# Andurdur/Chroma-Subsampling-Image-Compressor

Hardware: NVIDIA B200
Metric: input megapixels/s (higher is better)
Workload: dtype u8

## Files before the change

chroma-subsampling-image-compressor_b200/csrc/csic_flex_kernel.cu:

```cuda
#include <cuda_runtime.h>

#include <cstdint>
#include <type_traits>

#include "csic_internal.h"
#include "csic_device_math.cuh"
#include "csic_tma.cuh"

namespace csic {

namespace {

constexpr uint32_t kCtaWideSpan = 2048u;
constexpr uint32_t kDirectRowBytes = 257u;

__device__ __forceinline__ void sts64(uint32_t a, uint32_t x, uint32_t y) {
  asm volatile("st.shared.v2.u32 [%0], {%1, %2};" ::"r"(a), "r"(x), "r"(y) : "memory");
}
__device__ __forceinline__ void sts128(uint32_t a, uint32_t x, uint32_t y, uint32_t z, uint32_t w) {
  asm volatile("st.shared.v4.u32 [%0], {%1, %2, %3, %4};" ::"r"(a), "r"(x), "r"(y), "r"(z), "r"(w) : "memory");
}
__device__ __forceinline__ uint32_t ldg8_now(const uint8_t* p) {
  uint32_t v;
  asm volatile("ld.global.nc.u8 %0, [%1];" : "=r"(v) : "l"(p));
  return v;
}

__device__ __forceinline__ bool pow2_divides(uint32_t n, uint32_t m) {
  return n != 0u && (n & (n - 1u)) == 0u && (m & (m - 1u)) == 0u && n <= m;
}

template <typename F>
__device__ __forceinline__ void for_each_span(uint32_t n, uint32_t len, uint32_t NC, F&& fn) {
  const uint32_t tid = threadIdx.x, NW = NC >> 5;
  if ((len >= kCtaWideSpan || n == 1) && pow2_divides(n, NW)) {
    const uint32_t sh = 31u - __clz(NW) - (31u - __clz(n));
    const uint32_t parts = 1u << sh, j = (tid >> 5) >> sh, part = (tid >> 5) & (parts - 1u);
    fn(j, part * 32u + (tid & 31u), parts * 32u);
  } else if (len >= kCtaWideSpan || n == 1) {
    for (uint32_t j = 0; j < n; ++j) fn(j, tid, NC);
  } else {
    for (uint32_t j = tid >> 5; j < n; j += NW) fn(j, tid & 31u, 32u);
  }
}

__device__ __forceinline__ uint32_t lds_px(uint32_t a) {
  const uint32_t b = a & ~3u;
  return __funnelshift_r(lds32(b), lds32(b + 4), (a & 3u) * 8u);
}

template <uint32_t PXB>
__device__ __forceinline__ void load_granule_any(uint32_t a, uint32_t pxb, uint32_t (&p)[4]) {
  const uint32_t b = a & ~3u, sh = (a & 3u) * 8u;
  if (PXB == 3u) {
    const uint32_t w0 = lds32(b), w1 = lds32(b + 4), w2 = lds32(b + 8), w3 = lds32(b + 12);
    const uint32_t v0 = __funnelshift_r(w0, w1, sh), v1 = __funnelshift_r(w1, w2, sh), v2 = __funnelshift_r(w2, w3, sh);
    p[0] = v0;
    p[1] = __funnelshift_r(v0, v1, 24);
    p[2] = __funnelshift_r(v1, v2, 16);
    p[3] = v2 >> 8;
  } else if (PXB == 6u) {
    const uint32_t w0 = lds32(b), w1 = lds32(b + 4), w2 = lds32(b + 8), w3 = lds32(b + 12), w4 = lds32(b + 16), w5 = lds32(b + 20);
    p[0] = __funnelshift_r(w0, w1, sh);
    p[1] = __funnelshift_r(__funnelshift_r(w1, w2, sh), __funnelshift_r(w2, w3, sh), 16);
    p[2] = __funnelshift_r(w3, w4, sh);
    p[3] = __funnelshift_r(__funnelshift_r(w4, w5, sh), w5 >> sh, 16);
  } else {
#pragma unroll
    for (int j = 0; j < 4; ++j) p[j] = __funnelshift_r(lds32(b + j * pxb), lds32(b + j * pxb + 4), sh);
  }
}

template <int FMT> struct FlexFmt {
  static constexpr uint32_t kUnit = (FMT == KF_YCC888 || FMT == KF_RGB888) ? 12u : (FMT == KF_SLOT32 ? 16u : (FMT == KF_SLOT16 ? 8u : 4u));
};

struct FlexDesc {
  uint32_t k, ro0, nrows, col0;
  uint32_t npx, a0, gpr, last_px;
  uint32_t obase_lo, obase_hi, st_mul, st_add;
  uint32_t mode, sh, magic, n_gran;
  uint32_t row_out, out_one, ncols, direct;
};
static_assert(sizeof(FlexDesc) == kFlexDescBytes, "kFlexDescBytes out of sync");

}

template <int FMT, bool TRUNC, uint32_t HFE, uint32_t PXB, bool DIRECT>
__device__ __forceinline__ void flex_consume(const KPlan& P, uint8_t* smem, const Ring& ring) {
  constexpr uint32_t kUnit = FlexFmt<FMT>::kUnit;
  const uint32_t tid = threadIdx.x, NC = blockDim.x - 32u, NW = NC >> 5;
  const uint32_t sbase = smem_u32(smem), out_s = sbase + P.out_buf_off, held_base = sbase + P.meta_off;
  const uint32_t desc0 = sbase + P.bar_off + kRingBarBytes * ring.S;
  const uint32_t in_stage = P.stage_stride * (uint32_t)P.tile_rows + 32u;
  const uint32_t ipb = (uint32_t)P.in_px_bytes, pxb = (uint32_t)P.f * ipb;
  const uint32_t nsplit = (uint32_t)P.nsplit;
  const bool vhold = P.vf == 2;
  const uint32_t my = P.qmask & 0xFFu, mcb = (P.qmask >> 8) & 0xFFu, mcr = (P.qmask >> 16) & 0xFFu;
  const uint32_t qm0 = my | (mcb << 8) | (mcr << 16) | (my << 24);
  const uint32_t qm1 = mcb | (mcr << 8) | (my << 16) | (mcb << 24);
  const uint32_t qm2 = mcr | (my << 8) | (mcb << 16) | (mcr << 24);
  const int shy = 8 + P.sy, shb = 8 + P.scb, shr = 8 + P.scr, ly = P.cb_bits + P.cr_bits, lb = P.cr_bits;
  const bool q8 = FMT == KF_SLOT32 && P.sy == 0 && P.scb == 0 && P.scr == 0;
  const uint32_t vs_sh = P.planar_vs == 2 ? 1u : 0u, hs_sh = P.planar_hs == 4 ? 2u : (P.planar_hs == 2 ? 1u : 0u);
  const uint32_t rs_mul = P.in_dense ? P.in_row_bytes : P.stage_stride;
  const uint32_t rs_add = P.in_dense ? 0u : (((uint32_t)P.row_step * P.in_row_bytes) & 15u);

  Ring::Pos pos;
  for (uint32_t it = 0; it < ring.n_my; ++it, pos.next(ring.S)) {
    const uint32_t s = pos.s;
    ring.wait_full(pos);
    const uint32_t da = desc0 + s * kFlexDescBytes;
    const uint4 d0 = lds128(da), d1 = lds128(da + 16u), d2 = lds128(da + 32u), d3 = lds128(da + 48u);
    const uint4 d4 = lds128(da + 64u);
    const uint32_t Dk = d0.x, Dro0 = d0.y, Dnrows = d0.z, Dcol0 = d0.w, Dnpx = d1.x, Da0 = d1.y;
    constexpr bool direct = DIRECT;
    consumer_barrier(NC);

    const uint32_t in_s = sbase + s * in_stage, held_s = held_base + s * (uint32_t)kFlexMaxRows * 4u;
    const uint32_t gpr = d1.z, last_px = d1.w;
    uint8_t* obase = reinterpret_cast<uint8_t*>((uint64_t)d2.x | ((uint64_t)d2.y << 32));
    const uint32_t oa0 = d2.x, st_mul = d2.z, st_add = d2.w;
    uint8_t* fout = P.out + (uint64_t)Dk * P.out_frame_bytes;
    const uint32_t c_first = (Dro0 + (1u << vs_sh) - 1u) >> vs_sh;
    const uint32_t c_last1 = ((Dro0 + Dnrows - 1u) >> vs_sh) + 1u;
    const uint32_t nrc = (FMT == KF_PLANAR && c_last1 > c_first) ? c_last1 - c_first : 0u;
    const uint32_t ccols = (Dnpx + (1u << hs_sh) - 1u) >> hs_sh;
    const uint32_t cb_s = out_s + Dnrows * st_mul + 16u, cr_s = cb_s + nrc * ccols;

    auto granule = [&](uint32_t row, uint32_t g, uint32_t rs, uint32_t so_row, uint32_t hv) {
      const uint32_t c = g * 4u;
      uint32_t p[4], dy[4], xb[4], xr[4];
      if (c + 3u <= last_px) {
        load_granule_any<PXB>(rs + c * pxb, pxb, p);
      } else {
#pragma unroll
        for (int j = 0; j < 4; ++j) p[j] = lds_px(rs + min(c + j, last_px) * pxb);
      }
#pragma unroll
      for (int j = 0; j < 4; ++j) dy[j] = fwd_y16(p[j], P.coef_y);
      const uint32_t so = so_row + g * kUnit;
      uint8_t* gp = obase + (uint64_t)row * P.out_row_bytes + g * kUnit;
      const uint32_t gbytes = min(kUnit, d4.x - g * kUnit);
      if (FMT == KF_RGB888) {
        const uint32_t my8 = my << 8, mcb8 = mcb << 8, mcr8 = mcr << 8;
        auto emit = [&](const InvChroma& t0, const InvChroma& t1, const InvChroma& t2, const InvChroma& t3) {
          uint32_t w0, w1, w2;
        inv_granule(dy, my8, t0, t1, t2, t3, w0, w1, w2);
          if (direct) { const uint32_t ww[3] = {w0, w1, w2}; direct_store(gp, ww, gbytes); }
          else { sts32(so, w0); sts32(so + 4, w1); sts32(so + 8, w2); }
        };
        if (hv) {
          const InvChroma t = inv_chroma_terms(fwd_nc16<TRUNC>(hv & 0x00FFFFFFu, P.coef_ncb), fwd_nc16<TRUNC>(hv & 0x00FFFFFFu, P.coef_ncr), mcb8, mcr8);
          emit(t, t, t, t);
        } else {
          InvChroma t[4];
#pragma unroll
          for (int j = 0; j < 4; j += (int)HFE) t[j] = inv_chroma_terms(fwd_nc16<TRUNC>(p[j], P.coef_ncb), fwd_nc16<TRUNC>(p[j], P.coef_ncr), mcb8, mcr8);
          emit(t[0], t[1 - 1 % HFE], t[2 - 2 % HFE], t[3 - 3 % HFE]);
        }
        return;
      }
      if (hv) {
        const uint32_t hb = fwd_nc16<TRUNC>(hv & 0x00FFFFFFu, P.coef_ncb), hr = fwd_nc16<TRUNC>(hv & 0x00FFFFFFu, P.coef_ncr);
#pragma unroll
        for (int j = 0; j < 4; ++j) { xb[j] = hb; xr[j] = hr; }
      } else {
        xb[0] = fwd_nc16<TRUNC>(p[0], P.coef_ncb); xr[0] = fwd_nc16<TRUNC>(p[0], P.coef_ncr);
        if (HFE == 1) { xb[1] = fwd_nc16<TRUNC>(p[1], P.coef_ncb); xr[1] = fwd_nc16<TRUNC>(p[1], P.coef_ncr); }
        else { xb[1] = xb[0]; xr[1] = xr[0]; }
        if (HFE <= 2) { xb[2] = fwd_nc16<TRUNC>(p[2], P.coef_ncb); xr[2] = fwd_nc16<TRUNC>(p[2], P.coef_ncr); }
        else { xb[2] = xb[0]; xr[2] = xr[0]; }
        if (HFE == 1) { xb[3] = fwd_nc16<TRUNC>(p[3], P.coef_ncb); xr[3] = fwd_nc16<TRUNC>(p[3], P.coef_ncr); }
        else { xb[3] = xb[2]; xr[3] = xr[2]; }
      }
      if (FMT == KF_YCC888) {
        uint32_t t, u, ww[3];
        t = __byte_perm(dy[0], xb[0], 0x0051); u = __byte_perm(xr[0], dy[1], 0x0051);
        ww[0] = (__byte_perm(t, u, 0x5410) ^ 0x00FFFF00u) & qm0;
        t = __byte_perm(xb[1], xr[1], 0x0051); u = __byte_perm(dy[2], xb[2], 0x0051);
        ww[1] = (__byte_perm(t, u, 0x5410) ^ 0xFF00FFFFu) & qm1;
        t = __byte_perm(xr[2], dy[3], 0x0051); u = __byte_perm(xb[3], xr[3], 0x0051);
        ww[2] = (__byte_perm(t, u, 0x5410) ^ 0xFFFF00FFu) & qm2;
        if (direct) direct_store(gp, ww, gbytes);
        else { sts32(so, ww[0]); sts32(so + 4, ww[1]); sts32(so + 8, ww[2]); }
      } else if (FMT == KF_PLANAR) {
        const uint32_t my4 = my * 0x01010101u;
        sts32(so, __byte_perm(__byte_perm(dy[0], dy[1], 0x0051), __byte_perm(dy[2], dy[3], 0x0051), 0x5410) & my4);
        if (!hv) {
          const uint32_t crow = (((Dro0 + row) >> vs_sh) - c_first) * ccols + (c >> hs_sh);
          if (HFE == 1) {
#pragma unroll
            for (int j = 0; j < 4; ++j)
              if (c + j <= last_px) { sts8(cb_s + crow + j, (~(xb[j] >> 8)) & mcb); sts8(cr_s + crow + j, (~(xr[j] >> 8)) & mcr); }
          } else if (HFE == 2) {
            sts8(cb_s + crow, (~(xb[0] >> 8)) & mcb); sts8(cr_s + crow, (~(xr[0] >> 8)) & mcr);
            if (c + 2 <= last_px) { sts8(cb_s + crow + 1, (~(xb[2] >> 8)) & mcb); sts8(cr_s + crow + 1, (~(xr[2] >> 8)) & mcr); }
          } else {
            sts8(cb_s + crow, (~(xb[0] >> 8)) & mcb); sts8(cr_s + crow, (~(xr[0] >> 8)) & mcr);
          }
        }
      } else {
        uint32_t v[4];
        if (q8) {
#pragma unroll
          for (int j = 0; j < 4; ++j)
            v[j] = __byte_perm(__byte_perm(xr[j], xb[j], 0x0051), dy[j], 0x7510) ^ 0x0000FFFFu;
        } else {
#pragma unroll
          for (int j = 0; j < 4; ++j)
            v[j] = ((dy[j] >> shy) << ly) | (((xb[j] ^ 0xFFFFu) >> shb) << lb) | ((xr[j] ^ 0xFFFFu) >> shr);
        }
        if (c + 3u > last_px) {
#pragma unroll
          for (int j = 0; j < 4; ++j) if (c + j > last_px) v[j] = 0u;
        }
        if (direct) {
          if (FMT == KF_SLOT32) direct_store(gp, v, gbytes);
          else if (FMT == KF_SLOT16) { const uint32_t ww[2] = {v[0] | (v[1] << 16), v[2] | (v[3] << 16)}; direct_store(gp, ww, gbytes); }
          else { const uint32_t ww[1] = {v[0] | (v[1] << 8) | (v[2] << 16) | (v[3] << 24)}; direct_store(gp, ww, gbytes); }
        } else if (FMT == KF_SLOT32) {
          if ((so & 15u) == 0) sts128(so, v[0], v[1], v[2], v[3]);
          else if ((so & 7u) == 0) { sts64(so, v[0], v[1]); sts64(so + 8, v[2], v[3]); }
          else { sts32(so, v[0]); sts32(so + 4, v[1]); sts32(so + 8, v[2]); sts32(so + 12, v[3]); }
        } else if (FMT == KF_SLOT16) {
          if ((so & 7u) == 0) sts64(so, v[0] | (v[1] << 16), v[2] | (v[3] << 16));
          else { sts32(so, v[0] | (v[1] << 16)); sts32(so + 4, v[2] | (v[3] << 16)); }
        } else {
          sts32(so, v[0] | (v[1] << 8) | (v[2] << 16) | (v[3] << 24));
        }
      }
    };
    auto row_in = [&](uint32_t row) { return in_s + row * rs_mul + ((Da0 + row * rs_add) & 15u); };
    auto row_st = [&](uint32_t row) { return out_s + row * st_mul + ((oa0 + row * st_add) & 12u); };
    if (d3.x == 0u) {
      const uint32_t parts = 1u << d3.y, row = (tid >> 5) >> d3.y, part = (tid >> 5) & (parts - 1u);
      if (row < Dnrows) {
        const uint32_t rs = row_in(row), so_row = row_st(row), hv = vhold ? lds32(held_s + row * 4u) : 0u;
        for (uint32_t g = part * 32u + (tid & 31u); g < gpr; g += parts * 32u) granule(row, g, rs, so_row, hv);
      }
    } else if (d3.x == 1u) {
      for (uint32_t row = 0; row < Dnrows; ++row) {
        const uint32_t rs = row_in(row), so_row = row_st(row), hv = vhold ? lds32(held_s + row * 4u) : 0u;
        for (uint32_t g = tid; g < gpr; g += NC) granule(row, g, rs, so_row, hv);
      }
    } else if (d3.x == 2u) {
      for (uint32_t row = tid >> 5; row < Dnrows; row += NW) {
        const uint32_t rs = row_in(row), so_row = row_st(row), hv = vhold ? lds32(held_s + row * 4u) : 0u;
        for (uint32_t g = tid & 31u; g < gpr; g += 32u) granule(row, g, rs, so_row, hv);
      }
    } else {
      for (uint32_t q = tid; q < d3.w; q += NC) {
        const uint32_t row = gpr > 1u ? __umulhi(q, d3.z) : q, g = q - row * gpr;
        granule(row, g, row_in(row), row_st(row), vhold ? lds32(held_s + row * 4u) : 0u);
      }
    }
    consumer_barrier(NC);
    if (tid == 0) mbar_arrive(ring.empty(s));

    if (direct) {
    } else if (d4.y) {
      span_store(obase, out_s + (oa0 & 12u), Dnrows * d4.x, tid, NC);
    } else {
      for_each_span(Dnrows, d4.x, NC, [&](uint32_t j, uint32_t t, uint32_t n) {
        span_store(obase + (uint64_t)j * P.out_row_bytes, out_s + j * st_mul + ((oa0 + j * st_add) & 12u), d4.x, t, n);
      });
    }
    if (FMT == KF_PLANAR && nrc) {
      const uint64_t coff = (uint64_t)c_first * (uint32_t)P.planar_cw + (Dcol0 >> hs_sh);
      uint8_t* cb_g = fout + P.planar_cb_off + coff;
      uint8_t* cr_g = fout + P.planar_cr_off + coff;
      if (nsplit == 1) {
        span_store(cb_g, cb_s, nrc * ccols, tid, NC);
        span_store(cr_g, cr_s, nrc * ccols, tid, NC);
      } else {
        for_each_span(nrc, ccols, NC, [&](uint32_t j, uint32_t t, uint32_t n) {
          span_store(cb_g + (uint64_t)j * (uint32_t)P.planar_cw, cb_s + j * ccols, ccols, t, n);
          span_store(cr_g + (uint64_t)j * (uint32_t)P.planar_cw, cr_s + j * ccols, ccols, t, n);
        });
      }
    }
  }
}

template <int FMT, bool TRUNC>
__global__ void __launch_bounds__(kFlexMaxThreads, 4) csic_flex_kernel(const __grid_constant__ KPlan P) {
  extern __shared__ __align__(128) uint8_t smem[];
  constexpr uint32_t kUnit = FlexFmt<FMT>::kUnit, kOpx = kUnit / 4u;
  const uint32_t tid = threadIdx.x, NT = blockDim.x;
  const uint32_t sbase = smem_u32(smem), held_base = sbase + P.meta_off;
  const uint32_t in_stage = P.stage_stride * (uint32_t)P.tile_rows + 32u;
  const uint32_t ipb = (uint32_t)P.in_px_bytes, f = (uint32_t)P.f, pxb = f * ipb;
  const uint32_t nsplit = (uint32_t)P.nsplit;
  const uint32_t hfe = (uint32_t)P.hfe;
  const bool vhold = P.vf == 2;
  const uint64_t rstep = (uint64_t)(uint32_t)P.row_step * P.in_row_bytes;
  const Ring ring(sbase + P.bar_off, (uint32_t)P.stages, P.n_tiles);
  if (ring.n_my == 0) return;
  const uint32_t rs_mul = P.in_dense ? P.in_row_bytes : P.stage_stride;
  const uint32_t NC = NT - 32u;
  ring.init(1);

  if (tid >= NC) {
    const uint32_t lane = tid - NC;
    const uint64_t pol = policy_evict_first();
    const uint32_t t2 = blockIdx.x / nsplit, g2 = gridDim.x / nsplit;
    uint32_t pseg = blockIdx.x - t2 * nsplit, pk = t2 / P.tiles_per_band, ptb = t2 - pk * P.tiles_per_band;
    const uint32_t dseg = gridDim.x - g2 * nsplit, dk = g2 / P.tiles_per_band, dtb = g2 - dk * P.tiles_per_band;
    const uintptr_t lim_lo = reinterpret_cast<uintptr_t>(P.in) + (uint64_t)((uint32_t)P.row0 * (uint32_t)P.row_step) * P.in_row_bytes;
    const uintptr_t lim_hi = reinterpret_cast<uintptr_t>(P.in) + (uint64_t)(P.n_frames - 1u) * P.in_frame_bytes +
                             (uint64_t)((uint32_t)(P.row0 + P.band_rows - 1) * (uint32_t)P.row_step) * P.in_row_bytes +
                             ((uint32_t)P.Wo - 1u) * pxb + ipb;
    Ring::Pos pos;
    for (uint32_t j = 0; j < ring.n_my; ++j, pos.next(ring.S)) {
      const uint32_t s = pos.s, bar = ring.full(s), in_s = sbase + s * in_stage;
      ring.wait_empty(pos, j);
      FlexDesc* d = reinterpret_cast<FlexDesc*>(smem + P.bar_off + kRingBarBytes * ring.S) + s;
      const uint32_t ro0 = (uint32_t)P.row0 + ptb * (uint32_t)P.tile_rows;
      const uint32_t nrows = min((uint32_t)P.tile_rows, (uint32_t)(P.row0 + P.band_rows) - ro0);
      const uint32_t col0 = pseg * (uint32_t)P.tile_px;
      const uint32_t ncols = min((uint32_t)P.tile_px, (uint32_t)P.slots_per_row - col0);
      const uint32_t npx = min((uint32_t)P.Wo, col0 + ncols) - col0;
      const uint32_t len_in = (npx - 1u) * pxb + ipb;
      const uint8_t* frame = P.in + (uint64_t)pk * P.in_frame_bytes;
      const uint8_t* src0 = frame + (uint64_t)(ro0 * (uint32_t)P.row_step) * P.in_row_bytes + (uint64_t)col0 * pxb;
      uint32_t hw[kFlexMaxRows / 32];
#pragma unroll
      for (uint32_t u = 0; u < (uint32_t)kFlexMaxRows / 32u; ++u) {
        const uint32_t j = lane + 32u * u;
        uint32_t h0 = 0, h1 = 0, h2 = 0, hvalid = 0;
        if (vhold && j < nrows) {
          const uint32_t ro = ro0 + j;
          uint32_t rf = ro, fr0 = 0;
          if (P.tall_ho) { const uint32_t kf = ro / (uint32_t)P.tall_ho; fr0 = kf * (uint32_t)P.tall_ho; rf = ro - fr0; }
          const uint8_t* hp = nullptr;
          if (!P.case_b) {
            if (f == 1 && (rf & 1u)) hp = frame + (uint64_t)(ro - 1u) * P.in_row_bytes + (uint32_t)P.last_sample_col * ipb;
          } else {
            const uint32_t line = rf >> (31u - __clz(f));
            if (line & 1u) {
              const uint32_t srow = fr0 + (line - 1u) * f + P.caseb_row_add;
              hp = frame + (uint64_t)(srow * (uint32_t)P.row_step) * P.in_row_bytes + P.caseb_col_bytes;
            }
          }
          if (hp) { h0 = ldg8_now(hp); h1 = ldg8_now(hp + 1); h2 = ldg8_now(hp + 2); hvalid = 0x80000000u; }
        }
        hw[u] = hvalid ? (hvalid | h0 | (h1 << 8) | (h2 << 16)) : 0u;
      }
      if (lane == 0) {
        const uint32_t NWc = NC >> 5, gpr = (ncols + 3u) >> 2, srow = gpr * kUnit, row_out = ncols * kOpx;
        const uint64_t ob = reinterpret_cast<uint64_t>(P.out) + (uint64_t)pk * P.out_frame_bytes + (uint64_t)ro0 * P.out_row_bytes +
                            (uint64_t)col0 * kOpx;
        const uint32_t out_one = (P.out_dense && nsplit == 1u && row_out == srow) ? 1u : 0u;
        const uint32_t parts = nrows <= NWc ? NWc / nrows : 0u;
        uint32_t mode = 3u, sh = 0u;
        if (parts && (parts & (parts - 1u)) == 0u) {
          sh = 31u - __clz(parts);
          const uint32_t lsh = sh + 5u, iters = (gpr + (1u << lsh) - 1u) >> lsh;
          if (gpr * 5u >= (iters << lsh) * 4u) mode = 0u;
        }
        if (mode != 0u) {
          const uint32_t rounds = (nrows + NWc - 1u) / NWc, li = (gpr + 31u) >> 5;
          if (gpr >= 4u * NC) mode = 1u;
          else if (nrows > NWc && nrows * 5u >= rounds * NWc * 4u && gpr * 5u >= li * 32u * 4u) mode = 2u;
        }
        d->k = pk; d->ro0 = ro0; d->nrows = nrows; d->col0 = col0;
        d->npx = npx; d->a0 = (uint32_t)reinterpret_cast<uintptr_t>(src0) & 15u; d->gpr = gpr; d->last_px = npx - 1u;
        d->obase_lo = (uint32_t)ob; d->obase_hi = (uint32_t)(ob >> 32);
        d->st_mul = out_one ? srow : srow + 16u; d->st_add = out_one ? 0u : P.out_row_bytes;
        d->mode = mode; d->sh = sh; d->magic = gpr > 1u ? 0xFFFFFFFFu / gpr + 1u : 0u;
        d->n_gran = nrows * gpr;
        d->row_out = row_out; d->out_one = out_one; d->ncols = ncols;
        d->direct = 0u;
      }
      if (P.in_dense) {
        if (lane == 0) span_fetch(in_s, src0, (nrows - 1u) * P.in_row_bytes + len_in, bar, pol, lim_lo, lim_hi);
      } else {
        for (uint32_t j = lane; j < nrows; j += 32u)
          span_fetch(in_s + j * rs_mul, src0 + (uint64_t)j * rstep, len_in, bar, pol, lim_lo, lim_hi);
      }
      if (vhold) {
#pragma unroll
        for (uint32_t u = 0; u < (uint32_t)kFlexMaxRows / 32u; ++u)
          sts32(held_base + (s * (uint32_t)kFlexMaxRows + lane + 32u * u) * 4u, hw[u]);
      }
      __syncwarp();
      if (lane == 0) mbar_arrive(bar);
      pseg += dseg;
      uint32_t c = pseg >= nsplit ? 1u : 0u;
      pseg -= c * nsplit;
      ptb += dtb + c;
      c = ptb >= P.tiles_per_band ? 1u : 0u;
      ptb -= c * P.tiles_per_band;
      pk += dk + c;
    }
    return;
  }

  const uint32_t row_out_full = min((uint32_t)P.tile_px, (uint32_t)P.slots_per_row) * kOpx;
  const bool out_one_full = P.out_dense && nsplit == 1u && row_out_full == ((min((uint32_t)P.tile_px, (uint32_t)P.slots_per_row) + 3u) >> 2) * kUnit;
  const bool direct = FMT != KF_PLANAR && nsplit == 1u && !out_one_full && row_out_full < kDirectRowBytes;
  auto run = [&](auto hfe_tag) {
    constexpr uint32_t H = decltype(hfe_tag)::value;
    if (direct) {
      if (pxb == 3u) flex_consume<FMT, TRUNC, H, 3u, true>(P, smem, ring);
      else if (pxb == 6u) flex_consume<FMT, TRUNC, H, 6u, true>(P, smem, ring);
      else flex_consume<FMT, TRUNC, H, 0u, true>(P, smem, ring);
    } else if (pxb == 3u) flex_consume<FMT, TRUNC, H, 3u, false>(P, smem, ring);
    else if (pxb == 6u) flex_consume<FMT, TRUNC, H, 6u, false>(P, smem, ring);
    else flex_consume<FMT, TRUNC, H, 0u, false>(P, smem, ring);
  };
  if (hfe == 1u) run(std::integral_constant<uint32_t, 1u>{});
  else if (hfe == 2u) run(std::integral_constant<uint32_t, 2u>{});
  else run(std::integral_constant<uint32_t, 4u>{});
}

KernelFn flex_kernel(int kformat, bool trunc) {
  switch (kformat) {
    case KF_YCC888: return trunc ? csic_flex_kernel<KF_YCC888, true> : csic_flex_kernel<KF_YCC888, false>;
    case KF_RGB888: return trunc ? csic_flex_kernel<KF_RGB888, true> : csic_flex_kernel<KF_RGB888, false>;
    case KF_SLOT8: return trunc ? csic_flex_kernel<KF_SLOT8, true> : csic_flex_kernel<KF_SLOT8, false>;
    case KF_SLOT16: return trunc ? csic_flex_kernel<KF_SLOT16, true> : csic_flex_kernel<KF_SLOT16, false>;
    case KF_PLANAR: return trunc ? csic_flex_kernel<KF_PLANAR, true> : csic_flex_kernel<KF_PLANAR, false>;
    default: return trunc ? csic_flex_kernel<KF_SLOT32, true> : csic_flex_kernel<KF_SLOT32, false>;
  }
}

}
```

chroma-subsampling-image-compressor_b200/csrc/csic_internal.h:

```cpp
#ifndef CSIC_INTERNAL_H_
#define CSIC_INTERNAL_H_

#include <cstddef>
#include <cstdint>
#include <vector>

#include "../../include/csic.h"

namespace csic {

struct Geometry {
  int32_t out_w, out_h;
  size_t in_row_bytes, in_frame_bytes;
  size_t out_row_bytes, out_frame_bytes;
  int32_t out_px_bytes;
  int32_t in_px_bytes;
  bool chroma_first;
  bool quant_first;
  int32_t hf, vf;
  int32_t planar_hs, planar_vs, planar_cw, planar_ch;
};

int slot_bits(const csic_params& p);
Geometry geometry(const csic_params& p);

enum KFormat : int32_t { KF_YCC888 = 0, KF_RGB888 = 1, KF_SLOT8 = 2, KF_SLOT16 = 3, KF_SLOT32 = 4, KF_PLANAR = 5 };

struct KPlan {
  const uint8_t* in;
  uint8_t* out;
  uint64_t in_frame_bytes, out_frame_bytes;
  uint32_t in_row_bytes, out_row_bytes;
  int32_t W, H, Wo, Ho;
  int32_t Wp;
  int32_t in_dense, out_dense, ragged;
  int32_t in_px_bytes;
  uint32_t coef_y, coef_ncb, coef_ncr;
  int32_t f;
  int32_t hf, vf, last_sample_col;
  int32_t case_b;
  uint32_t caseb_row_add, caseb_col_bytes;
  int32_t quant_first, trunc, average;
  int32_t kformat, slot_bytes, slots_per_row;
  int32_t planar_hs, planar_vs, planar_cw, planar_ch;
  uint64_t planar_cb_off, planar_cr_off;
  int32_t sy, scb, scr;
  int32_t cb_bits, cr_bits;
  int32_t row0, band_rows;
  int32_t compact;
  int32_t row_step;
  uint32_t n_frames;
  int32_t hfe;
  int32_t nsplit, tile_px;
  int32_t tile_rows;
  uint32_t tiles_per_band;
  uint32_t tile_in_bytes, tile_out_bytes;
  uint32_t n_tiles;
  int32_t stages;
  int32_t block_threads;
  int32_t ctas_per_sm;
  uint32_t stage_stride, out_buf_off, out_buf_stride, meta_off, bar_off, smem_bytes;
  uint32_t qmask;
  int32_t tall_ho;
};

constexpr uint32_t kRingBarBytes = 16;
constexpr int kDefaultBlockThreads = 256;
constexpr int kMaxConsumerThreads = 512;
constexpr int kMaxTileRows = 64;
constexpr uint32_t kTileMetaBytes = 32 + 4 * kMaxTileRows;
constexpr int kPoolMaxRows = 16;
constexpr uint32_t kPoolMetaBytes = 32 + 4 * kPoolMaxRows;
constexpr int kFlexMaxRows = 64;
constexpr int kFlexConsumers = 256;
constexpr int kFlexMaxThreads = 288;
constexpr uint32_t kFlexTileBytes = 24u * 1024u;
constexpr uint32_t kFlexDescBytes = 80u;
constexpr int kDecConsumers = 256;
constexpr int kDecMaxConsumers = 512;
constexpr uint32_t kDecDescBytes = 48u;

struct DecPlan {
  const uint8_t* planar;
  uint8_t* out;
  uint64_t frame_bytes, cb_off, cr_off;
  uint64_t lim_lo, lim_hi;
  uint32_t Wo, Ho, A;
  uint32_t cw;
  uint32_t hs_sh, vhold, last_c;
  uint32_t tile_px, tiles_per_frame, n_tiles;
  uint32_t stages, y_slot, c_slot, stage_stride, out_off, out_stride, desc_off, bar_off;
  uint32_t to_rgb;
};

struct Layout {
  size_t in_pitch = 0, in_frame = 0, out_pitch = 0, out_frame = 0;
  bool short_frames = false;
};
int build_plan(const csic_params& p, const void* d_rgb, void* d_out, size_t n_frames, int32_t row0, int32_t rows,
               bool compact, const Layout& lay, KPlan& k);

struct DeviceLimits { int sm_count; size_t max_smem_optin; };
struct PlanOptions { int family = 0, stages = 0; uint32_t tile_bytes = 0; int block_threads = 0, ctas_per_sm = 0; };
enum Family : int32_t { FAM_GENERIC = 1, FAM_ROWS = 2, FAM_POOL = 3, FAM_FLEX = 4 };
struct KernelChoice { int32_t family; KPlan k; unsigned grid; };
KernelChoice select_kernel(const KPlan& base, const DeviceLimits& dev, const PlanOptions& opt);

constexpr int kPipe = 3;
struct CopySide { size_t off, pitch, frame; CopySide at(size_t k) const { return {off + k * frame, pitch, frame}; } };
struct CopyShape { size_t width, rows; CopySide caller, bounce, staging; };
struct HostPlan {
  bool compact;
  size_t first_stored;
  Layout lay;
  size_t in_pitch, out_pitch;
  size_t frames_per_chunk;
  CopyShape in, out;
};
int plan_host(const csic_params& p, int32_t row0, int32_t rows, size_t n_frames, const DeviceLimits& dev,
              const PlanOptions& opt, size_t chunk_bytes, bool full_frames, size_t share_gpus, HostPlan& h);
struct Copy { size_t dst, dst_pitch, src, src_pitch, width, height; };
std::vector<Copy> frame_copies(const CopyShape& s, const CopySide& dst, const CopySide& src, size_t nf);
void band_split(const csic_params& p, size_t i, size_t G, int32_t& r0, int32_t& r1);

struct DecodeLaunch { DecPlan P; unsigned grid, threads; size_t smem; };
bool plan_decode(const KPlan& k, int to_rgb, const DeviceLimits& dev, uint32_t tile_px, DecodeLaunch& d);

using KernelFn = void (*)(KPlan);
using DecodeFn = void (*)(DecPlan);
template <int F> KernelFn rows_kernel(int kformat, bool q8, bool trunc);
template <int F> KernelFn pool_kernel(int kformat, bool in4);
KernelFn flex_kernel(int kformat, bool trunc);
DecodeFn decode_kernel(uint32_t hs_sh, bool vhold, bool to_rgb);
int launch(const KernelChoice& c, void* stream);
int set_kernel_attributes(size_t max_smem_optin);
int launch_expand_planar(const KPlan& k, int to_rgb, int sm_count, void* stream);
int launch_decode_tma(const DecodeLaunch& d, void* stream);

}

#endif
```

chroma-subsampling-image-compressor_b200/csrc/csic_plan.cpp:

```cpp
#include <algorithm>
#include <cstring>

#include "csic_internal.h"

namespace csic {

namespace {

constexpr uint32_t kSmemPerSm = 227u * 1024u;

uint32_t up16(uint32_t v) { return (v + 15u) & ~15u; }
uint32_t up128(uint32_t v) { return (v + 127u) & ~127u; }
uint32_t ctas_by_smem(uint32_t smem) { return kSmemPerSm / (smem + 1024u); }

unsigned persistent_grid(uint64_t n_tiles, int sm_count, uint32_t per_sm) {
  return (unsigned)std::min<uint64_t>(n_tiles, (uint64_t)(uint32_t)sm_count * per_sm);
}

bool plan_case_b(KPlan& k, int wo_unit) {
  if (!k.case_b) return true;
  if (k.W % k.f != 0 || k.Wo % wo_unit != 0) return false;
  k.caseb_row_add = (uint32_t)k.last_sample_col / (uint32_t)k.Wo;
  k.caseb_col_bytes = ((uint32_t)k.last_sample_col % (uint32_t)k.Wo) * (uint32_t)k.in_px_bytes * (uint32_t)k.f;
  return true;
// ... 114 lines not shown
  if (planar)
    k.out_buf_stride = up128((uint32_t)rows * (uint32_t)k.tile_px +
                             2u * (uint32_t)((rows + k.planar_vs - 1) / k.planar_vs) * ((uint32_t)k.tile_px / (uint32_t)k.planar_hs));
  auto need = [&](int s) {
    return (uint32_t)s * k.stage_stride + 2u * k.out_buf_stride + (uint32_t)s * kTileMetaBytes + (uint32_t)s * 16u + 384u;
  };
  auto ctas_for = [&](int s) {
    return std::min<uint32_t>(std::min<uint32_t>(ctas_by_smem(need(s)), 2048u / ((uint32_t)k.block_threads + 32u)), 8u);
  };
  int stages = force_stages >= 2 ? force_stages : (k.f >= 4 ? 3 : 2);
  while (force_stages < 2 && stages > 2 && ctas_for(stages) < 2) --stages;
  if (need(stages) > max_smem_optin || ctas_for(stages) < 1) return false;
  k.ctas_per_sm = (int32_t)std::min<uint32_t>(ctas_for(stages), tiny ? 8u : (k.f == 1 ? 4u : 2u));
  k.stages = stages;
  if (tall) commit_tall(k);
  ring_layout(k, (uint32_t)stages, kTileMetaBytes);
  return true;
}

bool plan_pool_kernel(KPlan& k, int sm_count, size_t max_smem_optin) {
  const bool staged = k.kformat <= KF_RGB888;
  const uint32_t opx = staged ? 3u : (uint32_t)k.slot_bytes;
  if (!plan_case_b(k, k.hf) || !plan_padded_rows(k, opx)) return false;
  const bool auto_threads = k.block_threads <= 0;
  if (auto_threads) k.block_threads = k.f >= 4 ? 192 : kDefaultBlockThreads;
  if (k.block_threads > kMaxConsumerThreads) return false;

  const uint32_t f = (uint32_t)k.f, ipb = (uint32_t)k.in_px_bytes;
  const uint32_t budget = 24u * 1024u, tile_max = budget + budget / 3;
  const uint32_t block_row_bytes = (uint32_t)k.Wp * f * f * ipb;
  if (!plan_segments(k, block_row_bytes, tile_max, 16, 256)) return false;
  k.tile_in_bytes = (uint32_t)k.tile_px * f * f * ipb;
  k.tile_out_bytes = (uint32_t)k.tile_px * opx;
  int rows = 1;
  if (k.nsplit == 1) {
    rows = budget_rows(k.tile_in_bytes, budget, tile_max, 1 << 30);
    rows = std::min(rows, (int)(2u * (uint32_t)kPoolMaxRows / f));
    rows = std::min(rows, k.band_rows);
    if (!k.out_dense) rows = 1;
    rows = spread_rows(rows, k.n_frames, k.band_rows, sm_count);
    rows = std::min(rows, equal_tile_rows(rows, k.band_rows));
  }
  if (!plan_tiles(k, rows, k.n_frames, k.band_rows)) return false;
  const uint32_t units = (uint32_t)rows * ((uint32_t)k.tile_px >> 2) * 4u;
  const bool small_cta = auto_threads && k.f == 8 && 2u * units <= (uint32_t)k.block_threads;
  if (small_cta) k.block_threads = (int32_t)std::max(64u, (units + 31u) & ~31u);
  k.stage_stride = up128((uint32_t)rows * k.tile_in_bytes + (uint32_t)kPoolMaxRows * 32u);
  k.out_buf_stride = staged ? (uint32_t)(kMaxConsumerThreads / 32) * 384u / 2u : 0u;
  k.stages = 2;
  const uint32_t need = 2u * k.stage_stride + 2u * k.out_buf_stride + 2u * kPoolMetaBytes + 32u + 384u;
  if (need > max_smem_optin) return false;
  const uint32_t threads = (uint32_t)k.block_threads + 32u;
  const uint32_t by_regs = 65536u / ((k.f == 2 ? 56u : 72u) * threads);
  k.ctas_per_sm = (int32_t)std::max<uint32_t>(1u, std::min<uint32_t>(std::min<uint32_t>(small_cta ? 8u : 4u, by_regs), ctas_by_smem(need)));
  ring_layout(k, 2u, kPoolMetaBytes);
  return true;
}

bool plan_flex_kernel(KPlan& k, int sm_count, size_t max_smem_optin, int force_stages, uint32_t force_tile_bytes) {
  const uint32_t ipb = (uint32_t)k.in_px_bytes, f = (uint32_t)k.f, pxb = f * ipb;
  if (!plan_case_b(k, k.hf)) return false;
  k.hfe = hold_width(k);
  const bool planar = k.kformat == KF_PLANAR;
  const uint32_t unit = (k.kformat <= KF_RGB888) ? 12u : (planar ? 4u : 4u * (uint32_t)k.slot_bytes);
  const uint32_t S = (uint32_t)k.slots_per_row, Wo = (uint32_t)k.Wo;
  const uint32_t tile_bytes = force_tile_bytes ? std::max(1024u, force_tile_bytes) : kFlexTileBytes;
  const uint32_t tile_px_max = std::max(16u, (tile_bytes / pxb) & ~15u);
  k.tile_px = (int32_t)std::min(tile_px_max, (S + 15u) & ~15u);
  k.nsplit = (int32_t)((S + (uint32_t)k.tile_px - 1u) / (uint32_t)k.tile_px);
  const uint32_t len_in_max = ((std::min((uint32_t)k.tile_px, Wo) - 1u) * f + 1u) * ipb;
  const bool contiguous = k.nsplit == 1 && k.row_step == 1 && k.in_row_bytes == (uint32_t)k.W * ipb;
  if (k.block_threads <= 0) k.block_threads = kFlexConsumers;
  k.block_threads = std::min(k.block_threads, kFlexMaxThreads - 32);
  const uint32_t stages = (uint32_t)std::min(std::max(force_stages, 2), 8);

  const bool tall = batch_is_tall(k);
  const uint32_t frames = tall ? 1u : k.n_frames;
  const uint32_t band_rows = tall ? k.n_frames * (uint32_t)k.Ho : (uint32_t)k.band_rows;

  const uint32_t NW = (uint32_t)k.block_threads / 32u, gpr = (std::min((uint32_t)k.tile_px, S) + 3u) / 4u;
  const uint32_t row_in = up16((contiguous ? std::max(len_in_max, k.in_row_bytes) : len_in_max) + 15u) + 16u;
  uint32_t row_out = ((uint32_t)k.tile_px / 4u) * unit + 16u;
  if (planar) row_out += 2u * (uint32_t)k.tile_px;
  const uint32_t cta_cap = std::min<uint32_t>(std::min<uint32_t>(8u, 2048u / ((uint32_t)k.block_threads + 32u)),
                                              65536u / (56u * ((uint32_t)k.block_threads + 32u)));
  auto ctas_for = [&](uint32_t r) {
    const uint32_t smem = stages * (r * row_in + 32u) + r * row_out + 2048u;
    return std::min<uint32_t>(cta_cap, ctas_by_smem(smem));
  };
  int rows = 1;
  if (k.nsplit == 1) {
    const uint32_t rmax = std::min<uint32_t>((uint32_t)kFlexMaxRows, band_rows);
    auto tiles_for = [&](uint32_t r) { return (uint64_t)frames * (uint64_t)((band_rows + r - 1u) / r); };
    if (force_tile_bytes) {
      const uint32_t per_row = contiguous ? k.in_row_bytes : len_in_max;
      rows = (int)std::min<uint32_t>(rmax, std::max<uint32_t>(1u, tile_bytes / std::max(1u, per_row)));
    } else {
      auto busy_frac = [&](uint32_t r) {
        const bool lanes_ok = gpr * 5u >= ((gpr + 31u) / 32u) * 32u * 4u;
        if (r <= NW) {
          const uint32_t parts = NW / r;
          const uint32_t lanes = parts * 32u, it = (gpr + lanes - 1u) / lanes;
          if ((parts & (parts - 1u)) == 0u && gpr * 5u >= it * lanes * 4u) return (double)(r * parts) / NW;
          return 0.85;
        }
        const uint32_t rounds = (r + NW - 1u) / NW;
        if (lanes_ok && r * 5u >= rounds * NW * 4u) return (double)r / (rounds * NW);
        return 0.85;
      };
      const double busy_cap = k.kformat == KF_RGB888 ? 32.0 : 20.0;
      double best_score = -1.0;
      for (uint32_t r = 1; r <= rmax; ++r) {
        const uint32_t c = ctas_for(r);
        if (c == 0u) break;
        if (r > 1u && tiles_for(r) < (uint64_t)sm_count * 8u) break;
        const double gran = (double)r * gpr;
        const double fill = (double)band_rows / (double)(((band_rows + r - 1u) / r) * r);
        const double score = std::min(busy_cap, c * NW * busy_frac(r)) * gran / (gran + 400.0) * (c >= 3u ? 1.0 : 0.85) * fill;
        if (score >= best_score * 1.0001) { best_score = score; rows = (int)r; }
      }
    }
  }
  if (!plan_tiles(k, rows, frames, (int)band_rows)) return false;
  k.in_dense = (contiguous && rows > 1) ? 1 : 0;
  const uint32_t dense_out_row = planar ? Wo : S * (unit / 4u);
  k.out_dense = k.out_row_bytes == dense_out_row ? 1 : 0;

  k.stage_stride = row_in;
  const uint32_t in_bytes = stages * ((uint32_t)rows * k.stage_stride + 32u);
  uint32_t stage_bytes = (uint32_t)rows * (((uint32_t)k.tile_px / 4u) * unit + 16u) + 16u;
  if (planar) stage_bytes += 2u * (uint32_t)(rows / std::max(1, k.planar_vs) + 1) * (uint32_t)k.tile_px;
  k.out_buf_off = up128(in_bytes);
  k.out_buf_stride = up16(stage_bytes + 32u);
  k.meta_off = k.out_buf_off + k.out_buf_stride;
  k.bar_off = up128(k.meta_off + stages * (uint32_t)kFlexMaxRows * 4u);
  k.smem_bytes = k.bar_off + stages * (kRingBarBytes + kFlexDescBytes);
  if (k.smem_bytes > max_smem_optin) return false;
  k.tall_ho = tall ? k.Ho : 0;
  if (tall) commit_tall(k);
  k.stages = (int32_t)stages;
  k.ctas_per_sm = (int32_t)std::max<uint32_t>(1u, std::min<uint32_t>(cta_cap, ctas_by_smem(k.smem_bytes)));
  return true;
}

unsigned generic_grid(const KPlan& k, int sm_count) {
  const uint64_t n_rows = (uint64_t)k.n_frames * (uint64_t)k.band_rows;
  if (n_rows == 0 || k.slots_per_row == 0) return 0;
  const uint32_t gpr = ((uint32_t)k.slots_per_row + 3u) >> 2;
  const uint64_t groups = gpr < 32u ? (n_rows + 32u / gpr - 1u) / (32u / gpr) : n_rows;
  return (unsigned)std::min<uint64_t>((groups + 3u) / 4u, (uint64_t)sm_count * 16u);
}

}

int build_plan(const csic_params& p, const void* d_rgb, void* d_out, size_t n_frames, int32_t row0,
               int32_t rows, bool compact, const Layout& lay, KPlan& k) {
  const Geometry g = geometry(p);
  std::memset(&k, 0, sizeof(k));
  k.in = static_cast<const uint8_t*>(d_rgb);
  k.out = static_cast<uint8_t*>(d_out);
  k.compact = compact ? 1 : 0;
  k.row_step = compact ? 1 : p.factor;
  k.in_frame_bytes = compact ? g.in_row_bytes * (size_t)g.out_h : g.in_frame_bytes;
  k.out_frame_bytes = g.out_frame_bytes;
  if (g.in_row_bytes > 0xFFFFFFFFull || g.out_row_bytes > 0xFFFFFFFFull) return CSIC_EINVAL_DIMS;
  if ((uint64_t)g.out_w * (uint64_t)g.out_h >= (1ull << 31) || (uint64_t)p.width * p.height >= (1ull << 31))
    return CSIC_EINVAL_DIMS;
  k.in_row_bytes = (uint32_t)g.in_row_bytes;
  k.out_row_bytes = (uint32_t)g.out_row_bytes;
  if (lay.in_pitch) {
    if (lay.in_pitch < g.in_row_bytes || lay.in_pitch > 0xFFFFFFFFull) return CSIC_EINVAL_ARG;
    k.in_row_bytes = (uint32_t)lay.in_pitch;
    k.in_frame_bytes = (size_t)lay.in_pitch * (size_t)(compact ? g.out_h : p.height);
  }
  if (lay.in_frame) {
    if (lay.in_frame < k.in_frame_bytes && !lay.short_frames) return CSIC_EINVAL_ARG;
    k.in_frame_bytes = lay.in_frame;
  }
  if ((lay.out_pitch || lay.out_frame || lay.short_frames) && p.out_format == CSIC_OUT_PLANAR)
    return CSIC_EINVAL_MODE;
  if (lay.out_pitch) {
    if (lay.out_pitch < g.out_row_bytes || lay.out_pitch > 0xFFFFFFFFull) return CSIC_EINVAL_ARG;
    k.out_row_bytes = (uint32_t)lay.out_pitch;
    k.out_frame_bytes = (size_t)lay.out_pitch * (size_t)g.out_h;
  }
  if (lay.out_frame) {
    if (lay.out_frame < k.out_frame_bytes && !lay.short_frames) return CSIC_EINVAL_ARG;
    k.out_frame_bytes = lay.out_frame;
  }
  k.in_px_bytes = g.in_px_bytes;
  auto swap_rb = [](uint32_t c) { return (c & 0xFF00FF00u) | ((c & 0xFFu) << 16) | ((c >> 16) & 0xFFu); };
  const bool bgr = p.in_format == CSIC_IN_BGRA32;
  k.coef_y = bgr ? swap_rb(0x001D964Du) : 0x001D964Du;
  k.coef_ncb = bgr ? swap_rb(0x0080552Bu) : 0x0080552Bu;
  k.coef_ncr = bgr ? swap_rb(0x00156B80u) : 0x00156B80u;
  k.W = p.width;
  k.H = p.height;
  k.Wo = g.out_w;
  k.Ho = g.out_h;
  k.f = p.factor;
  k.hf = g.hf;
  k.vf = g.vf;
  k.last_sample_col = ((p.width - 1) / g.hf) * g.hf;
  k.case_b = (!g.chroma_first && p.factor > 1 && (g.hf > 1 || g.vf > 1)) ? 1 : 0;
  k.quant_first = g.quant_first ? 1 : 0;
  k.trunc = p.round_mode == CSIC_ROUND_TRUNC;
  k.average = (p.pool_mode == CSIC_POOL_AVERAGE && p.factor > 1) ? 1 : 0;
  if (p.out_format == CSIC_OUT_YCC888) k.kformat = KF_YCC888;
  else if (p.out_format == CSIC_OUT_RGB888) k.kformat = KF_RGB888;
  else if (p.out_format == CSIC_OUT_PLANAR) k.kformat = KF_PLANAR;
  else k.kformat = g.out_px_bytes == 1 ? KF_SLOT8 : (g.out_px_bytes == 2 ? KF_SLOT16 : KF_SLOT32);
  k.slot_bytes = g.out_px_bytes;
  k.slots_per_row = (k.kformat <= KF_RGB888 || k.kformat == KF_PLANAR)
                        ? g.out_w : (int32_t)(g.out_row_bytes / (size_t)g.out_px_bytes);
  k.planar_hs = g.planar_hs; k.planar_vs = g.planar_vs; k.planar_cw = g.planar_cw; k.planar_ch = g.planar_ch;
  k.planar_cb_off = (uint64_t)g.out_w * (uint64_t)g.out_h;
  k.planar_cr_off = k.planar_cb_off + (uint64_t)g.planar_cw * (uint64_t)g.planar_ch;
// ... 194 lines not shown
```

Baseline: 2.664 million.

## Move flex kernel output stores to producer-issued TMA bulk stores with ring staging

After: 2.667 million, median of 6. No clear change (+0.1%).

```diff
diff --git a/chroma-subsampling-image-compressor_b200/csrc/csic_flex_kernel.cu b/chroma-subsampling-image-compressor_b200/csrc/csic_flex_kernel.cu
--- a/chroma-subsampling-image-compressor_b200/csrc/csic_flex_kernel.cu
+++ b/chroma-subsampling-image-compressor_b200/csrc/csic_flex_kernel.cu
@@ -12,7 +12,6 @@
 namespace {
 
 constexpr uint32_t kCtaWideSpan = 2048u;
-constexpr uint32_t kDirectRowBytes = 257u;
 
 __device__ __forceinline__ void sts64(uint32_t a, uint32_t x, uint32_t y) {
   asm volatile("st.shared.v2.u32 [%0], {%1, %2};" ::"r"(a), "r"(x), "r"(y) : "memory");
@@ -20,6 +19,55 @@
 __device__ __forceinline__ void sts128(uint32_t a, uint32_t x, uint32_t y, uint32_t z, uint32_t w) {
   asm volatile("st.shared.v4.u32 [%0], {%1, %2, %3, %4};" ::"r"(a), "r"(x), "r"(y), "r"(z), "r"(w) : "memory");
 }
+__device__ __forceinline__ void sts16(uint32_t a, uint32_t v) {
+  asm volatile("st.shared.u16 [%0], %1;" ::"r"(a), "h"((unsigned short)v) : "memory");
+}
+__device__ __forceinline__ uint32_t lds16(uint32_t a) {
+  unsigned short v;
+  asm volatile("ld.shared.u16 %0, [%1];" : "=h"(v) : "r"(a));
+  return v;
+}
+
+__device__ __forceinline__ void sts_gran12(uint32_t a, uint32_t w0, uint32_t w1, uint32_t w2) {
+  switch (a & 3u) {
+    case 0u: sts32(a, w0); sts32(a + 4, w1); sts32(a + 8, w2); break;
+    case 1u:
+      sts8(a, w0); sts16(a + 1, w0 >> 8);
+      sts32(a + 3, __funnelshift_r(w0, w1, 24)); sts32(a + 7, __funnelshift_r(w1, w2, 24));
+      sts8(a + 11, w2 >> 24);
+      break;
+    case 2u:
+      sts16(a, w0);
+      sts32(a + 2, __funnelshift_r(w0, w1, 16)); sts32(a + 6, __funnelshift_r(w1, w2, 16));
+      sts16(a + 10, w2 >> 16);
+      break;
+    default:
+      sts8(a, w0);
+      sts32(a + 1, __funnelshift_r(w0, w1, 8)); sts32(a + 5, __funnelshift_r(w1, w2, 8));
+      sts16(a + 9, w2 >> 8); sts8(a + 11, w2 >> 24);
+      break;
+  }
+}
+
+__device__ __forceinline__ void edge_copy(uint8_t* g, uint32_t s, uint32_t n) {
+  for (uint32_t i = 0; i < n;) {
+    const uint32_t a = s + i, left = n - i;
+    if ((a & 7u) == 0 && left >= 8u) { *reinterpret_cast<uint2*>(g + i) = lds64(a); i += 8u; }
+    else if ((a & 3u) == 0 && left >= 4u) { *reinterpret_cast<uint32_t*>(g + i) = lds32(a); i += 4u; }
+    else if ((a & 1u) == 0 && left >= 2u) { *reinterpret_cast<unsigned short*>(g + i) = (unsigned short)lds16(a); i += 2u; }
+    else { g[i] = (uint8_t)lds8(a); i += 1u; }
+  }
+}
+
+__device__ __forceinline__ void span_store_bulk(uint8_t* g, uint32_t s, uint32_t len, uint64_t pol) {
+  const uintptr_t A = reinterpret_cast<uintptr_t>(g), B = A + len;
+  const uintptr_t up = (A + 15u) & ~(uintptr_t)15, dn = B & ~(uintptr_t)15;
+  const uintptr_t lo = up < B ? up : B, hi = dn > lo ? dn : lo;
+  if (hi > lo) tma_store_1d(reinterpret_cast<void*>(lo), s + (uint32_t)(lo - A), (uint32_t)(hi - lo), pol);
+  edge_copy(g, s, (uint32_t)(lo - A));
+  edge_copy(reinterpret_cast<uint8_t*>(hi), s + (uint32_t)(hi - A), (uint32_t)(B - hi));
+}
+
 __device__ __forceinline__ uint32_t ldg8_now(const uint8_t* p) {
   uint32_t v;
   asm volatile("ld.global.nc.u8 %0, [%1];" : "=r"(v) : "l"(p));
@@ -80,7 +128,7 @@
   uint32_t npx, a0, gpr, last_px;
   uint32_t obase_lo, obase_hi, st_mul, st_add;
   uint32_t mode, sh, magic, n_gran;
-  uint32_t row_out, out_one, ncols, direct;
+  uint32_t row_out, out_one, in_s, stg;
 };
 static_assert(sizeof(FlexDesc) == kFlexDescBytes, "kFlexDescBytes out of sync");
 
@@ -90,7 +138,9 @@
 __device__ __forceinline__ void flex_consume(const KPlan& P, uint8_t* smem, const Ring& ring) {
   constexpr uint32_t kUnit = FlexFmt<FMT>::kUnit;
   const uint32_t tid = threadIdx.x, NC = blockDim.x - 32u, NW = NC >> 5;
-  const uint32_t sbase = smem_u32(smem), out_s = sbase + P.out_buf_off, held_base = sbase + P.meta_off;
+  constexpr bool kBulk = (FMT == KF_YCC888 || FMT == KF_RGB888) && !DIRECT;
+  constexpr uint32_t kStMask = kBulk ? 15u : 12u;
+  const uint32_t sbase = smem_u32(smem), held_base = sbase + P.meta_off;
   const uint32_t desc0 = sbase + P.bar_off + kRingBarBytes * ring.S;
   const uint32_t in_stage = P.stage_stride * (uint32_t)P.tile_rows + 32u;
   const uint32_t ipb = (uint32_t)P.in_px_bytes, pxb = (uint32_t)P.f * ipb;
@@ -115,9 +165,10 @@
     const uint4 d4 = lds128(da + 64u);
     const uint32_t Dk = d0.x, Dro0 = d0.y, Dnrows = d0.z, Dcol0 = d0.w, Dnpx = d1.x, Da0 = d1.y;
     constexpr bool direct = DIRECT;
-    consumer_barrier(NC);
-
-    const uint32_t in_s = sbase + s * in_stage, held_s = held_base + s * (uint32_t)kFlexMaxRows * 4u;
+    if (!kBulk) consumer_barrier(NC);
+
+    const uint32_t in_s = kBulk ? d4.z : sbase + s * in_stage, out_s = kBulk ? d4.w : sbase + P.out_buf_off;
+    const uint32_t held_s = held_base + s * (uint32_t)kFlexMaxRows * 4u;
     const uint32_t gpr = d1.z, last_px = d1.w;
     uint8_t* obase = reinterpret_cast<uint8_t*>((uint64_t)d2.x | ((uint64_t)d2.y << 32));
     const uint32_t oa0 = d2.x, st_mul = d2.z, st_add = d2.w;
@@ -148,7 +199,7 @@
           uint32_t w0, w1, w2;
         inv_granule(dy, my8, t0, t1, t2, t3, w0, w1, w2);
           if (direct) { const uint32_t ww[3] = {w0, w1, w2}; direct_store(gp, ww, gbytes); }
-          else { sts32(so, w0); sts32(so + 4, w1); sts32(so + 8, w2); }
+          else sts_gran12(so, w0, w1, w2);
         };
         if (hv) {
           const InvChroma t = inv_chroma_terms(fwd_nc16<TRUNC>(hv & 0x00FFFFFFu, P.coef_ncb), fwd_nc16<TRUNC>(hv & 0x00FFFFFFu, P.coef_ncr), mcb8, mcr8);
@@ -183,7 +234,7 @@
         t = __byte_perm(xr[2], dy[3], 0x0051); u = __byte_perm(xb[3], xr[3], 0x0051);
         ww[2] = (__byte_perm(t, u, 0x5410) ^ 0xFFFF00FFu) & qm2;
         if (direct) direct_store(gp, ww, gbytes);
-        else { sts32(so, ww[0]); sts32(so + 4, ww[1]); sts32(so + 8, ww[2]); }
+        else sts_gran12(so, ww[0], ww[1], ww[2]);
       } else if (FMT == KF_PLANAR) {
         const uint32_t my4 = my * 0x01010101u;
         sts32(so, __byte_perm(__byte_perm(dy[0], dy[1], 0x0051), __byte_perm(dy[2], dy[3], 0x0051), 0x5410) & my4);
@@ -232,7 +283,7 @@
       }
     };
     auto row_in = [&](uint32_t row) { return in_s + row * rs_mul + ((Da0 + row * rs_add) & 15u); };
-    auto row_st = [&](uint32_t row) { return out_s + row * st_mul + ((oa0 + row * st_add) & 12u); };
+    auto row_st = [&](uint32_t row) { return out_s + row * st_mul + ((oa0 + row * st_add) & kStMask); };
     if (d3.x == 0u) {
       const uint32_t parts = 1u << d3.y, row = (tid >> 5) >> d3.y, part = (tid >> 5) & (parts - 1u);
       if (row < Dnrows) {
@@ -255,10 +306,11 @@
         granule(row, g, row_in(row), row_st(row), vhold ? lds32(held_s + row * 4u) : 0u);
       }
     }
+    if (kBulk) fence_proxy_async_smem();
     consumer_barrier(NC);
     if (tid == 0) mbar_arrive(ring.empty(s));
 
-    if (direct) {
+    if (direct || kBulk) {
     } else if (d4.y) {
       span_store(obase, out_s + (oa0 & 12u), Dnrows * d4.x, tid, NC);
     } else {
@@ -304,6 +356,9 @@
   if (tid >= NC) {
     const uint32_t lane = tid - NC;
     const uint64_t pol = policy_evict_first();
+    const bool bulk = (FMT == KF_YCC888 || FMT == KF_RGB888) && P.flex_out >= FLEX_BULK_STAGE;
+    const bool rot = bulk && P.flex_out == FLEX_BULK_REGION;
+    const uint32_t R = ring.S + (rot ? 1u : 0u);
     const uint32_t t2 = blockIdx.x / nsplit, g2 = gridDim.x / nsplit;
     uint32_t pseg = blockIdx.x - t2 * nsplit, pk = t2 / P.tiles_per_band, ptb = t2 - pk * P.tiles_per_band;
     const uint32_t dseg = gridDim.x - g2 * nsplit, dk = g2 / P.tiles_per_band, dtb = g2 - dk * P.tiles_per_band;
@@ -312,10 +367,25 @@
                              (uint64_t)((uint32_t)(P.row0 + P.band_rows - 1) * (uint32_t)P.row_step) * P.in_row_bytes +
                              ((uint32_t)P.Wo - 1u) * pxb + ipb;
     Ring::Pos pos;
-    for (uint32_t j = 0; j < ring.n_my; ++j, pos.next(ring.S)) {
-      const uint32_t s = pos.s, bar = ring.full(s), in_s = sbase + s * in_stage;
+    uint32_t r = 0;
+    for (uint32_t j = 0; j < ring.n_my + (bulk ? ring.S : 0u); ++j, pos.next(ring.S), r = r + 1u == R ? 0u : r + 1u) {
+      const uint32_t s = pos.s, bar = ring.full(s), in_s = sbase + (rot ? r : s) * in_stage;
       ring.wait_empty(pos, j);
       FlexDesc* d = reinterpret_cast<FlexDesc*>(smem + P.bar_off + kRingBarBytes * ring.S) + s;
+      if (bulk && j >= ring.S) {
+        const uint64_t ob = (uint64_t)d->obase_lo | ((uint64_t)d->obase_hi << 32);
+        const uint32_t stg = d->stg, nr = d->nrows, len = d->row_out, st_mul = d->st_mul, st_add = d->st_add;
+        if (d->out_one) {
+          if (lane == 0) span_store_bulk(reinterpret_cast<uint8_t*>(ob), stg + ((uint32_t)ob & 15u), nr * len, pol);
+        } else {
+          for (uint32_t i = lane; i < nr; i += 32u)
+            span_store_bulk(reinterpret_cast<uint8_t*>(ob + (uint64_t)i * P.out_row_bytes), stg + i * st_mul + (((uint32_t)ob + i * st_add) & 15u),
+                            len, pol);
+        }
+        tma_store_commit();
+        __syncwarp();
+      }
+      if (j >= ring.n_my) continue;
       const uint32_t ro0 = (uint32_t)P.row0 + ptb * (uint32_t)P.tile_rows;
       const uint32_t nrows = min((uint32_t)P.tile_rows, (uint32_t)(P.row0 + P.band_rows) - ro0);
       const uint32_t col0 = pseg * (uint32_t)P.tile_px;
@@ -367,11 +437,19 @@
         d->k = pk; d->ro0 = ro0; d->nrows = nrows; d->col0 = col0;
         d->npx = npx; d->a0 = (uint32_t)reinterpret_cast<uintptr_t>(src0) & 15u; d->gpr = gpr; d->last_px = npx - 1u;
         d->obase_lo = (uint32_t)ob; d->obase_hi = (uint32_t)(ob >> 32);
-        d->st_mul = out_one ? srow : srow + 16u; d->st_add = out_one ? 0u : P.out_row_bytes;
+        d->st_mul = out_one ? srow : (bulk ? (srow + 30u) & ~15u : srow + 16u); d->st_add = out_one ? 0u : P.out_row_bytes;
         d->mode = mode; d->sh = sh; d->magic = gpr > 1u ? 0xFFFFFFFFu / gpr + 1u : 0u;
         d->n_gran = nrows * gpr;
-        d->row_out = row_out; d->out_one = out_one; d->ncols = ncols;
-        d->direct = 0u;
+        d->row_out = row_out; d->out_one = out_one;
+        if (bulk) {
+          d->in_s = in_s;
+          d->stg = sbase + (rot ? (r == 0u ? R - 1u : r - 1u) * in_stage : P.out_buf_off + s * P.out_buf_stride);
+        }
+      }
+      if (rot) {
+        tma_store_wait_read0();
+        fence_proxy_async_smem();
+        __syncwarp();
       }
       if (P.in_dense) {
         if (lane == 0) span_fetch(in_s, src0, (nrows - 1u) * P.in_row_bytes + len_in, bar, pol, lim_lo, lim_hi);
@@ -384,6 +462,7 @@
         for (uint32_t u = 0; u < (uint32_t)kFlexMaxRows / 32u; ++u)
           sts32(held_base + (s * (uint32_t)kFlexMaxRows + lane + 32u * u) * 4u, hw[u]);
       }
+      if (bulk && !rot) tma_store_wait_read0();
       __syncwarp();
       if (lane == 0) mbar_arrive(bar);
       pseg += dseg;
@@ -394,12 +473,11 @@
       ptb -= c * P.tiles_per_band;
       pk += dk + c;
     }
+    if (bulk) tma_store_wait_all();
     return;
   }
 
-  const uint32_t row_out_full = min((uint32_t)P.tile_px, (uint32_t)P.slots_per_row) * kOpx;
-  const bool out_one_full = P.out_dense && nsplit == 1u && row_out_full == ((min((uint32_t)P.tile_px, (uint32_t)P.slots_per_row) + 3u) >> 2) * kUnit;
-  const bool direct = FMT != KF_PLANAR && nsplit == 1u && !out_one_full && row_out_full < kDirectRowBytes;
+  const bool direct = FMT != KF_PLANAR && P.flex_out == FLEX_DIRECT;
   auto run = [&](auto hfe_tag) {
     constexpr uint32_t H = decltype(hfe_tag)::value;
     if (direct) {
diff --git a/chroma-subsampling-image-compressor_b200/csrc/csic_internal.h b/chroma-subsampling-image-compressor_b200/csrc/csic_internal.h
--- a/chroma-subsampling-image-compressor_b200/csrc/csic_internal.h
+++ b/chroma-subsampling-image-compressor_b200/csrc/csic_internal.h
@@ -62,7 +62,10 @@
   uint32_t stage_stride, out_buf_off, out_buf_stride, meta_off, bar_off, smem_bytes;
   uint32_t qmask;
   int32_t tall_ho;
+  int32_t flex_out;
 };
+
+enum FlexOut : int32_t { FLEX_SPAN = 0, FLEX_DIRECT = 1, FLEX_BULK_STAGE = 2, FLEX_BULK_REGION = 3 };
 
 constexpr uint32_t kRingBarBytes = 16;
 constexpr int kDefaultBlockThreads = 256;
@@ -76,6 +79,7 @@
 constexpr int kFlexMaxThreads = 288;
 constexpr uint32_t kFlexTileBytes = 24u * 1024u;
 constexpr uint32_t kFlexDescBytes = 80u;
+constexpr uint32_t kDirectRowBytes = 257u;
 constexpr int kDecConsumers = 256;
 constexpr int kDecMaxConsumers = 512;
 constexpr uint32_t kDecDescBytes = 48u;
diff --git a/chroma-subsampling-image-compressor_b200/csrc/csic_plan.cpp b/chroma-subsampling-image-compressor_b200/csrc/csic_plan.cpp
--- a/chroma-subsampling-image-compressor_b200/csrc/csic_plan.cpp
+++ b/chroma-subsampling-image-compressor_b200/csrc/csic_plan.cpp
@@ -220,10 +220,20 @@
   const uint32_t row_in = up16((contiguous ? std::max(len_in_max, k.in_row_bytes) : len_in_max) + 15u) + 16u;
   uint32_t row_out = ((uint32_t)k.tile_px / 4u) * unit + 16u;
   if (planar) row_out += 2u * (uint32_t)k.tile_px;
+  const uint32_t dense_out_row = planar ? Wo : S * (unit / 4u);
+  k.out_dense = k.out_row_bytes == dense_out_row ? 1 : 0;
+  const uint32_t row_out_full = std::min((uint32_t)k.tile_px, S) * (unit / 4u);
+  const bool out_one_full = k.out_dense && k.nsplit == 1 && row_out_full == gpr * unit;
+  const bool direct = !planar && k.nsplit == 1 && !out_one_full && row_out_full < kDirectRowBytes;
+  const bool bulk = k.kformat <= KF_RGB888 && !direct;
+  const uint32_t row_slot = up16(gpr * unit + 15u);
+  auto region_of = [&](uint32_t r) { return r * row_in + 32u; };
+  auto by_region = [&](uint32_t r) { return region_of(r) <= stages * r * row_slot; };
   const uint32_t cta_cap = std::min<uint32_t>(std::min<uint32_t>(8u, 2048u / ((uint32_t)k.block_threads + 32u)),
                                               65536u / (56u * ((uint32_t)k.block_threads + 32u)));
   auto ctas_for = [&](uint32_t r) {
-    const uint32_t smem = stages * (r * row_in + 32u) + r * row_out + 2048u;
+    const uint32_t out = !bulk ? r * row_out : (by_region(r) ? region_of(r) : stages * r * row_slot);
+    const uint32_t smem = stages * region_of(r) + out + 2048u;
     return std::min<uint32_t>(cta_cap, ctas_by_smem(smem));
   };
   int rows = 1;
@@ -261,16 +271,19 @@
   }
   if (!plan_tiles(k, rows, frames, (int)band_rows)) return false;
   k.in_dense = (contiguous && rows > 1) ? 1 : 0;
-  const uint32_t dense_out_row = planar ? Wo : S * (unit / 4u);
-  k.out_dense = k.out_row_bytes == dense_out_row ? 1 : 0;
 
   k.stage_stride = row_in;
-  const uint32_t in_bytes = stages * ((uint32_t)rows * k.stage_stride + 32u);
-  uint32_t stage_bytes = (uint32_t)rows * (((uint32_t)k.tile_px / 4u) * unit + 16u) + 16u;
-  if (planar) stage_bytes += 2u * (uint32_t)(rows / std::max(1, k.planar_vs) + 1) * (uint32_t)k.tile_px;
-  k.out_buf_off = up128(in_bytes);
-  k.out_buf_stride = up16(stage_bytes + 32u);
-  k.meta_off = k.out_buf_off + k.out_buf_stride;
+  k.flex_out = direct ? FLEX_DIRECT : !bulk ? FLEX_SPAN : by_region((uint32_t)rows) ? FLEX_BULK_REGION : FLEX_BULK_STAGE;
+  k.out_buf_off = up128((stages + (k.flex_out == FLEX_BULK_REGION ? 1u : 0u)) * region_of((uint32_t)rows));
+  if (bulk) {
+    k.out_buf_stride = k.flex_out == FLEX_BULK_STAGE ? (uint32_t)rows * row_slot : 0u;
+    k.meta_off = k.out_buf_off + stages * k.out_buf_stride;
+  } else {
+    uint32_t stage_bytes = (uint32_t)rows * (((uint32_t)k.tile_px / 4u) * unit + 16u) + 16u;
+    if (planar) stage_bytes += 2u * (uint32_t)(rows / std::max(1, k.planar_vs) + 1) * (uint32_t)k.tile_px;
+    k.out_buf_stride = up16(stage_bytes + 32u);
+    k.meta_off = k.out_buf_off + k.out_buf_stride;
+  }
   k.bar_off = up128(k.meta_off + stages * (uint32_t)kFlexMaxRows * 4u);
   k.smem_bytes = k.bar_off + stages * (kRingBarBytes + kFlexDescBytes);
   if (k.smem_bytes > max_smem_optin) return false;
```
